# SilvioWeging/kASA

Measured on AMD Instinct MI355X. Metric: reads/s in identify (10M x 150bp vs k=12 index), higher is better.
Workload: dtype u64

## Files before the change

### kasa_amd/csrc/kasa_hip.hip

```cpp
#include <hip/hip_runtime.h>
#include <chrono>
#include <cstdlib>
#include <cstring>
#include <rocprim/device/device_radix_sort.hpp>
#include <rocprim/device/device_segmented_radix_sort.hpp>
#include <rocprim/iterator/transform_iterator.hpp>
#include <rocprim/device/device_scan.hpp>
#include <rocprim/functional.hpp>
#include <rocprim/iterator/counting_iterator.hpp>

#include <algorithm>
#include <cstdarg>
#include <cstdint>
#include <cstdio>
#include <cstring>
#include <map>
#include <mutex>
#include <new>
#include <string>
#include <thread>
#include <type_traits>
#include <vector>

#include <dlfcn.h>
// ... 1531 lines not shown
        if (p >= nQ) continue;
        const Key q = qv[it];
        uint32_t lo;
        Key eLo = 0, ePrev = 0;
        bool hasLo, hasPrev;
        if (staged) {
            const uint32_t a = pos[it];
            lo = ilo + a;
            hasLo = a < span; hasPrev = a > 0;
            if (hasLo) eLo = sIdx[a];
            if (hasPrev) ePrev = sIdx[a - 1];
            if (!hasPrev && lo > 0) { ePrev = idxKmer[lo - 1]; hasPrev = true; }
            if (!hasLo && lo < nIdx) { eLo = idxKmer[lo]; hasLo = true; }
        } else {
            lo = lower_bound_global<Key>(idxKmer, table, tb, q);
            hasLo = lo < nIdx; hasPrev = lo > 0;
            if (hasLo) eLo = idxKmer[lo];
            if (hasPrev) ePrev = idxKmer[lo - 1];
        }
        const Key xa = hasLo ? (q ^ eLo) : ~(Key)0;
        const Key xb = hasPrev ? (q ^ ePrev) : ~(Key)0;
        const int la = lcp_of_xor<Key>(xa);
        int L = lcp_of_xor<Key>(xa < xb ? xa : xb);
        const uint32_t r = (la == L) ? lo : lo - 1;
        int d = 0;
        if (L >= RANGE_LETTERS) {
            d = L > kHigh ? kHigh : L;
            const Key x = q ^ HAT_ALL;
            const Key z = ~(((x & LOW4_ALL) + LOW4_ALL) | x) & BIT4_ALL & hatLetters;
            if (z) {
                const int khat = KLETTERS - ((int)(8 * sizeof(Key)) - 5 - clz_key(z)) / 5;
                if (khat <= d) d = khat - 1;
            }
            if (d < kLow) d = 0;
        }
        outD[it] = (uint32_t)d;
        outRep[it] = r;
        const Key prevQ = it ? qv[it - 1] : qBefore;
        const int ql = (p == 0) ? 0 : lcp_letters<Key>(prevQ, q);
        uint32_t m = allLv;
        if (ql >= RANGE_LETTERS) m = (d > ql) ? ((((2u << (d - ql - 1)) - 1u) << (kHigh - d)) & allLv) : 0u;
        special[it] = m;
    }
    const uint32_t anySpecial = special[0] | special[1] | special[2] | special[3];
    for (int lv = 0; lv < nK; ++lv) {
        const bool has = (anySpecial >> lv) & 1u;
        const unsigned long long mk = __ballot(has);
        if (has && (mk & ((1ull << (tid & 63)) - 1ull)) == 0ull) {
            const uint32_t it = ((special[0] >> lv) & 1u) ? 0u : ((special[1] >> lv) & 1u) ? 1u : ((special[2] >> lv) & 1u) ? 2u : 3u;
            atomicMin(&sFirst[lv], p0 + it);
        }
    }
    if (fullTile) {
        *reinterpret_cast<uint4 *>(rep + p0) = make_uint4(outRep[0], outRep[1], outRep[2], outRep[3]);
        *reinterpret_cast<uchar4 *>(depth + p0) = make_uchar4((uint8_t)outD[0], (uint8_t)outD[1], (uint8_t)outD[2], (uint8_t)outD[3]);
    } else {
#pragma unroll
        for (int it = 0; it < ITEMS; ++it)
            if (p0 + it < nQ) { rep[p0 + it] = outRep[it]; depth[p0 + it] = (uint8_t)outD[it]; }
    }
    __syncthreads();
    if (tid < nK) tileFirst[(size_t)tid * nTiles + blockIdx.x] = sFirst[tid];
}

__device__ __forceinline__ void suffix_min_1024(uint32_t *sh, uint32_t v, uint32_t &excl, uint32_t &all)
{
    sh[threadIdx.x] = v;
    __syncthreads();
    for (int off = 1; off < 1024; off <<= 1) {
        const uint32_t o = (threadIdx.x >= (unsigned)off) ? sh[threadIdx.x - off] : NOPOS;
        __syncthreads();
        if (o < sh[threadIdx.x]) sh[threadIdx.x] = o;
        __syncthreads();
    }
    excl = (threadIdx.x == 0) ? NOPOS : sh[threadIdx.x - 1];
    all = sh[1023];
    __syncthreads();
}

__global__ __launch_bounds__(1024) void tile_suffix_local_kernel(const uint32_t *__restrict__ tileFirst, uint32_t *__restrict__ tileNext,
                                                                 uint32_t *__restrict__ chunkMin, uint32_t nTiles, uint32_t nChunks)
{
    __shared__ uint32_t sh[1024];
    const uint32_t lv = blockIdx.y, chunk = blockIdx.x;
    const uint64_t end = std::min<uint64_t>((uint64_t)(chunk + 1) * 1024u, nTiles);
    const int64_t t = (int64_t)end - 1 - threadIdx.x;
    const bool in = t >= (int64_t)chunk * 1024;
    uint32_t excl, all;
    suffix_min_1024(sh, in ? tileFirst[(size_t)lv * nTiles + t] : NOPOS, excl, all);
    if (in) tileNext[(size_t)lv * nTiles + t] = excl;
    if (threadIdx.x == 0) chunkMin[(size_t)lv * nChunks + chunk] = all;
}

__global__ __launch_bounds__(1024) void tile_suffix_kernel(const uint32_t *__restrict__ in0, uint32_t *__restrict__ out0,
                                                           uint32_t n, uint32_t last)
{
    __shared__ uint32_t sh[1024];
    const int lv = blockIdx.x;
    const uint32_t *in = in0 + (size_t)lv * n;
    uint32_t *out = out0 + (size_t)lv * n;
    uint32_t carry = last;
    for (int64_t hiT = (int64_t)n; hiT > 0; hiT -= 1024) {
        const int64_t t = hiT - 1 - threadIdx.x;
        uint32_t excl, all;
        suffix_min_1024(sh, (t >= 0) ? in[t] : NOPOS, excl, all);
        if (t >= 0) out[t] = excl < carry ? excl : carry;
        if (all < carry) carry = all;
    }
}

__global__ void tile_suffix_apply_kernel(uint32_t *__restrict__ tileNext, const uint32_t *__restrict__ chunkNext, uint32_t nTiles, uint32_t nChunks)
{
    const uint32_t t = blockIdx.x * blockDim.x + threadIdx.x, lv = blockIdx.y;
    if (t >= nTiles) return;
    const size_t at = (size_t)lv * nTiles + t;
    if (tileNext[at] == NOPOS) tileNext[at] = chunkNext[(size_t)lv * nChunks + (t >> 10)];
}

static int tile_suffix(kasa_ctx *c, uint32_t nTiles)
{
    if (nTiles == 0) return KASA_OK;
    const uint32_t nChunks = (nTiles + 1023u) / 1024u;
    int rc = c->tileChunks.reserve((size_t)2 * c->nK * nChunks * 4 + 64);
    if (rc) return rc;
    uint32_t *chunkMin = c->tileChunks.as<uint32_t>(), *chunkNext = chunkMin + (size_t)c->nK * nChunks;
    tile_suffix_local_kernel<<<dim3(nChunks, (unsigned)c->nK), 1024, 0, c->stream>>>(c->tileFirst.as<uint32_t>(), c->tileNext.as<uint32_t>(), chunkMin, nTiles, nChunks);
    tile_suffix_kernel<<<c->nK, 1024, 0, c->stream>>>(chunkMin, chunkNext, nChunks, (uint32_t)c->nQ);
    tile_suffix_apply_kernel<<<dim3(blocks_for(nTiles, 256), (unsigned)c->nK), 256, 0, c->stream>>>(c->tileNext.as<uint32_t>(), chunkNext, nTiles, nChunks);
    HIPCHK(hipGetLastError());
    return KASA_OK;
}

template <class Key>
__global__ void unique_flag_kernel(const Key *__restrict__ kmer, const uint32_t *__restrict__ read, uint32_t n, uint32_t *__restrict__ flag)
{
    const uint32_t i = blockIdx.x * blockDim.x + threadIdx.x;
    if (i < n) flag[i] = (i == 0 || kmer[i] != kmer[i - 1] || read[i] != read[i - 1]) ? 1u : 0u;
}

__global__ void read_count_kernel(const uint32_t *__restrict__ read, uint32_t n, uint64_t *__restrict__ cnt)
{
    const uint32_t i = blockIdx.x * blockDim.x + threadIdx.x;
    if (i < n) atomicAdd((unsigned long long *)&cnt[read[i]], 1ull);
}

template <class Key>
__global__ void unique_scatter_kernel(const Key *__restrict__ kmer, const uint32_t *__restrict__ read, uint32_t n,
                                      const uint32_t *__restrict__ slot, Key *__restrict__ outKmer, uint32_t *__restrict__ outRead)
{
    const uint32_t i = blockIdx.x * blockDim.x + threadIdx.x;
    if (i >= n) return;
    const uint32_t sl = slot[i];
    if (i == 0 || sl != slot[i - 1]) { outKmer[sl - 1] = kmer[i]; outRead[sl - 1] = read[i]; }
}

__global__ void slot_to_read_kernel(const uint32_t *__restrict__ slot, uint32_t n, const uint64_t *__restrict__ kmerOff, uint32_t nReads,
                                    uint32_t *__restrict__ read)
{
    const uint32_t i = blockIdx.x * blockDim.x + threadIdx.x;
    if (i >= n) return;
    const uint64_t s = slot[i];
    uint32_t lo = 0, hi = nReads;
    while (hi - lo > 1) { const uint32_t mid = lo + ((hi - lo) >> 1); if (kmerOff[mid] <= s) lo = mid; else hi = mid; }
    read[i] = lo;
}

template <class Key> static int lookup_part(kasa_ctx *c);

static constexpr unsigned SORT_TOP = 32, SORT_TOP_OLD = 40;
static constexpr uint32_t SORT_BUCKET_LIMIT = 1024;
static constexpr uint32_t SORT_BIG_CAP = 1u << 18;
static constexpr uint32_t SORT_BIG_LONGEST = 1u << 20;
static constexpr uint32_t RANK_TILE = 2048, RANK_HALO = 128;
template <class Key>
__global__ __launch_bounds__(256) void bucket_rank_kernel(const Key *__restrict__ kin, const uint32_t *__restrict__ vin, Key *__restrict__ kout,
                                                          uint32_t *__restrict__ vout, uint32_t n, int shift, uint32_t *__restrict__ big,
                                                          uint32_t *__restrict__ bigHead)
{
    constexpr uint32_t WIN = RANK_TILE + 2 * RANK_HALO;
    static_assert(WIN % 256 == 0, "whole wavefronts stage the window");
    __shared__ Key sK[WIN];
    __shared__ uint64_t sHead[WIN / 64];
    const uint32_t base = blockIdx.x * RANK_TILE;
    const uint32_t lo = base >= RANK_HALO ? base - RANK_HALO : 0u;
    const uint32_t hi = (uint64_t)base + RANK_TILE + RANK_HALO < (uint64_t)n ? base + RANK_TILE + RANK_HALO : n;
    const uint32_t win = hi - lo;
    for (uint32_t x = threadIdx.x; x < WIN; x += 256u) {
        bool head = false;
        if (x < win) {
            const uint32_t q = lo + x;
            const Key k = kin[q];
            head = q == 0u || (uint64_t)(kin[q - 1u] >> shift) != (uint64_t)(k >> shift);
            sK[x] = k;
        }
        const uint64_t m = __ballot(head);
        if ((threadIdx.x & 63u) == 0u) sHead[x >> 6] = m;
    }
    __syncthreads();
    const uint32_t lastWord = (win - 1u) >> 6;
    for (uint32_t e = threadIdx.x; e < RANK_TILE; e += 256u) {
        const uint32_t p = base + e;
        if (p >= n) break;
        const uint32_t i0 = p - lo, bit = i0 & 63u;
        const Key k = sK[i0];
        bool edge = false;
        uint32_t m = i0 >> 6;
        uint64_t w = sHead[m] & (~0ull >> (63u - bit));
        while (w == 0ull && m > 0u) w = sHead[--m];
        uint32_t hs = 0;
        if (w == 0ull) edge = true; else hs = m * 64u + 63u - (uint32_t)__clzll((long long)w);
        m = i0 >> 6;
        w = sHead[m] & ((~0ull << bit) << 1);
        while (w == 0ull && m < lastWord) w = sHead[++m];
        uint32_t he = win;
        if (w == 0ull) edge = edge || (hi < n); else he = m * 64u + (uint32_t)__ffsll((unsigned long long)w) - 1u;
        uint32_t L = i0 - hs, members = he - hs, rank = 0;
        if (!edge && members <= SORT_BUCKET_LIMIT) {
            for (uint32_t j = hs; j < i0; ++j) rank += (sK[j] <= k) ? 1u : 0u;
            for (uint32_t j = i0 + 1u; j < he; ++j) rank += (sK[j] < k) ? 1u : 0u;
        }
        if (edge) {
            const uint64_t top = (uint64_t)(k >> shift);
            uint32_t R = 0;
            rank = 0; L = 0;
            for (uint32_t q = p; q > 0 && L < SORT_BUCKET_LIMIT;) { --q; const Key o = kin[q]; if ((uint64_t)(o >> shift) != top) break; ++L; rank += (o <= k) ? 1u : 0u; }
            for (uint32_t q = p + 1; q < n && R < SORT_BUCKET_LIMIT; ++q) { const Key o = kin[q]; if ((uint64_t)(o >> shift) != top) break; ++R; rank += (o < k) ? 1u : 0u; }
            members = L + R + 1u;
        }
        if (members > SORT_BUCKET_LIMIT) {
            kout[p] = k; vout[p] = vin[p];
            if (L == 0u) { const uint32_t at = atomicAdd(big, 1u); if (at < SORT_BIG_CAP) bigHead[at] = p; }
        } else { const uint32_t at = p - L + rank; kout[at] = k; vout[at] = vin[p]; }
    }
}

__global__ __launch_bounds__(256) void bucket_rank32_kernel(const uint64_t *__restrict__ kin, const uint32_t *__restrict__ vin, uint64_t *__restrict__ kout,
                                                            uint32_t *__restrict__ vout, uint32_t n, int shift, uint32_t *__restrict__ big,
                                                            uint32_t *__restrict__ bigHead)
{
    constexpr uint32_t WIN = RANK_TILE + 2 * RANK_HALO, POS_BITS = 12;
    static_assert(WIN % 256 == 0 && WIN <= (1u << POS_BITS), "window positions fit the low bits of the LDS word; whole wavefronts stage it");
    __shared__ uint32_t sW[WIN + 1];
    __shared__ uint64_t sHead[WIN / 64];
    const uint32_t base = blockIdx.x * RANK_TILE;
    const uint32_t lo = base >= RANK_HALO ? base - RANK_HALO : 0u;
    const uint32_t hi = (uint64_t)base + RANK_TILE + RANK_HALO < (uint64_t)n ? base + RANK_TILE + RANK_HALO : n;
    const uint32_t win = hi - lo;
    const uint32_t lowMask = (1u << shift) - 1u;
    for (uint32_t x = threadIdx.x; x < WIN; x += 256u) {
        bool head = false;
        if (x < win) {
            const uint32_t q = lo + x;
            const uint64_t k = kin[q];
            head = q == 0u || (kin[q - 1u] >> shift) != (k >> shift);
            sW[x] = (((uint32_t)k & lowMask) << POS_BITS) | x;
        }
        const uint64_t m = __ballot(head);
        if ((threadIdx.x & 63u) == 0u) sHead[x >> 6] = m;
    }
    __syncthreads();
    const uint32_t lastWord = (win - 1u) >> 6;
    for (uint32_t e = threadIdx.x; e < RANK_TILE; e += 256u) {
        const uint32_t p = base + e;
        if (p >= n) break;
        const uint32_t i0 = p - lo, my = sW[i0], bit = i0 & 63u;
        bool edge = false;
        uint32_t m = i0 >> 6;
        uint64_t w = sHead[m] & (~0ull >> (63u - bit));
        while (w == 0ull && m > 0u) w = sHead[--m];
        uint32_t hs = 0;
        if (w == 0ull) edge = true; else hs = m * 64u + 63u - (uint32_t)__clzll((long long)w);
        m = i0 >> 6;
        w = sHead[m] & ((~0ull << bit) << 1);
        while (w == 0ull && m < lastWord) w = sHead[++m];
        uint32_t he = win;
        if (w == 0ull) edge = edge || (hi < n); else he = m * 64u + (uint32_t)__ffsll((unsigned long long)w) - 1u;
        uint32_t L = i0 - hs, members = he - hs, rank = 0;
        if (!edge && members <= SORT_BUCKET_LIMIT) {
            for (uint32_t j = hs; j < he; j += 2u) {
                const uint32_t a = sW[j], b = sW[j + 1u];
                rank += (a < my ? 1u : 0u) + ((j + 1u < he && b < my) ? 1u : 0u);
            }
        }
        const uint64_t k = kin[p];
        if (edge) {
            const uint64_t top = k >> shift;
            uint32_t R = 0;
            rank = 0; L = 0;
            for (uint32_t q = p; q > 0 && L < SORT_BUCKET_LIMIT;) { --q; const uint64_t o = kin[q]; if ((o >> shift) != top) break; ++L; rank += (o <= k) ? 1u : 0u; }
            for (uint32_t q = p + 1; q < n && R < SORT_BUCKET_LIMIT; ++q) { const uint64_t o = kin[q]; if ((o >> shift) != top) break; ++R; rank += (o < k) ? 1u : 0u; }
            members = L + R + 1u;
        }
        if (members > SORT_BUCKET_LIMIT) {
            kout[p] = k; vout[p] = vin[p];
            if (L == 0u) { const uint32_t at = atomicAdd(big, 1u); if (at < SORT_BIG_CAP) bigHead[at] = p; }
        } else { const uint32_t at = p - L + rank; kout[at] = k; vout[at] = vin[p]; }
    }
}

__global__ __launch_bounds__(256) void bucket_rank64_kernel(const uint64_t *__restrict__ kin, const uint32_t *__restrict__ vin, uint64_t *__restrict__ kout,
                                                            uint32_t *__restrict__ vout, uint32_t n, int shift, uint32_t *__restrict__ big,
                                                            uint32_t *__restrict__ bigHead)
{
    constexpr uint32_t WIN = RANK_TILE + 2 * RANK_HALO, POS_BITS = 12;
    static_assert(WIN % 256 == 0 && WIN <= (1u << POS_BITS), "window positions fit the low bits of the LDS word; whole wavefronts stage it");
    __shared__ __attribute__((aligned(16))) uint64_t sW[WIN + 2];
    __shared__ uint64_t sHead[WIN / 64];
    const uint32_t base = blockIdx.x * RANK_TILE;
    const uint32_t lo = base >= RANK_HALO ? base - RANK_HALO : 0u;
    const uint32_t hi = (uint64_t)base + RANK_TILE + RANK_HALO < (uint64_t)n ? base + RANK_TILE + RANK_HALO : n;
    const uint32_t win = hi - lo;
    const uint64_t lowMask = (1ull << shift) - 1ull;
    for (uint32_t x = threadIdx.x; x < WIN; x += 256u) {
        bool head = false;
        if (x < win) {
            const uint32_t q = lo + x;
            const uint64_t k = kin[q];
            head = q == 0u || (kin[q - 1u] >> shift) != (k >> shift);
            sW[x] = ((k & lowMask) << POS_BITS) | x;
        }
        const uint64_t m = __ballot(head);
        if ((threadIdx.x & 63u) == 0u) sHead[x >> 6] = m;
    }
    __syncthreads();
    const uint32_t lastWord = (win - 1u) >> 6;
    for (uint32_t e = threadIdx.x; e < RANK_TILE; e += 256u) {
        const uint32_t p = base + e;
        if (p >= n) break;
        const uint32_t i0 = p - lo, bit = i0 & 63u;
        const uint64_t my = sW[i0];
        bool edge = false;
        uint32_t m = i0 >> 6;
        uint64_t w = sHead[m] & (~0ull >> (63u - bit));
        while (w == 0ull && m > 0u) w = sHead[--m];
        uint32_t hs = 0;
        if (w == 0ull) edge = true; else hs = m * 64u + 63u - (uint32_t)__clzll((long long)w);
        m = i0 >> 6;
        w = sHead[m] & ((~0ull << bit) << 1);
        while (w == 0ull && m < lastWord) w = sHead[++m];
        uint32_t he = win;
        if (w == 0ull) edge = edge || (hi < n); else he = m * 64u + (uint32_t)__ffsll((unsigned long long)w) - 1u;
        uint32_t L = i0 - hs, members = he - hs, rank = 0;
        if (!edge && members <= SORT_BUCKET_LIMIT) {
            uint32_t j = hs;
            if (j & 1u) { rank += sW[j] < my ? 1u : 0u; ++j; }
            for (; j + 1u < he; j += 2u) {
                const ulonglong2 ab = *reinterpret_cast<const ulonglong2 *>(&sW[j]);
                rank += (ab.x < my ? 1u : 0u) + (ab.y < my ? 1u : 0u);
            }
            if (j < he) rank += sW[j] < my ? 1u : 0u;
        }
        const uint64_t k = kin[p];
        if (edge) {
            const uint64_t top = k >> shift;
            uint32_t R = 0;
            rank = 0; L = 0;
            for (uint32_t q = p; q > 0 && L < SORT_BUCKET_LIMIT;) { --q; const uint64_t o = kin[q]; if ((o >> shift) != top) break; ++L; rank += (o <= k) ? 1u : 0u; }
            for (uint32_t q = p + 1; q < n && R < SORT_BUCKET_LIMIT; ++q) { const uint64_t o = kin[q]; if ((o >> shift) != top) break; ++R; rank += (o < k) ? 1u : 0u; }
            members = L + R + 1u;
        }
        if (members > SORT_BUCKET_LIMIT) {
            kout[p] = k; vout[p] = vin[p];
            if (L == 0u) { const uint32_t at = atomicAdd(big, 1u); if (at < SORT_BIG_CAP) bigHead[at] = p; }
        } else { const uint32_t at = p - L + rank; kout[at] = k; vout[at] = vin[p]; }
    }
}

template <class Key>
__global__ void bucket_bounds_kernel(const Key *__restrict__ kin, uint32_t n, int shift, const uint32_t *__restrict__ head, uint32_t nHead,
                                     uint32_t *__restrict__ begin, uint32_t *__restrict__ end, uint32_t *__restrict__ longest)
{
    const uint32_t x = blockIdx.x * blockDim.x + threadIdx.x;
    if (x >= nHead) return;
    const uint32_t p = head[x];
    const uint64_t top = (uint64_t)(kin[p] >> shift);
    uint32_t lo = p, hi = n;
    while (lo < hi) { const uint32_t mid = lo + ((hi - lo) >> 1); if ((uint64_t)(kin[mid] >> shift) <= top) lo = mid + 1; else hi = mid; }
    begin[x] = p; end[x] = lo;
    atomicMax(longest, lo - p);
}

template <class Key>
static int sort_and_range_impl(kasa_ctx *c, int unique)
{
    c->grouped = false; c->slotOf = nullptr;
    HIPCHK(hipSetDevice(c->ix->device));
    uint64_t nQ = c->nQ;
    int rc;
    if ((rc = c->qKmerB.reserve(nQ * sizeof(Key) + 64)) || (rc = c->qReadB.reserve(nQ * 4 + 64))) return rc;
    Span stage(c, c->timers[KASA_STAGE_SORT]); if ((rc = stage.begin())) return rc;
    if (nQ > 0) {
        const unsigned BITS = (unsigned)KeyTraits<Key>::BITS;
        auto radix = [&](DevBuf &kIn, DevBuf &vIn, DevBuf &kOut, DevBuf &vOut, unsigned lo, unsigned hi) -> int {
            return dev_sort_pairs(c->sortTmp, c->stream, kIn.as<Key>(), kOut.as<Key>(), vIn.as<uint32_t>(), vOut.as<uint32_t>(), (size_t)nQ, lo, hi);
        };
        if (c->debugFlags & 64) {
            if ((rc = radix(c->qKmerA, c->qReadA, c->qKmerB, c->qReadB, 0u, BITS))) return rc;
        } else {
            const unsigned top = ((sizeof(Key) == 8) != ((c->debugFlags & 2097152) != 0)) ? SORT_TOP : SORT_TOP_OLD;
            uint32_t *big = &c->ctr()->sortBig.count, *longest = &c->ctr()->sortBig.longest;
            if ((rc = c->sortBig.reserve((size_t)SORT_BIG_CAP * 12 + 64))) return rc;
            uint32_t *bigHead = c->sortBig.as<uint32_t>(), *segBegin = bigHead + SORT_BIG_CAP, *segEnd = segBegin + SORT_BIG_CAP;
            if (c->debugFlags & 512) {
                if ((rc = radix(c->qKmerA, c->qReadA, c->qKmerB, c->qReadB, BITS - top, BITS))) return rc;
            } else {
                if ((rc = c->sortTmp.reserve(kasa_radix::scratch_bytes<Key>(nQ)))) return rc;
                Key *kRes; uint32_t *vRes;
                Span passes(c, c->kernels[KASA_KERNEL_SORT_PASSES]); if ((rc = passes.begin())) return rc;
                HIPCHK(kasa_radix::sort_pairs<Key>(c->qKmerA.as<Key>(), c->qReadA.as<uint32_t>(), c->qKmerB.as<Key>(), c->qReadB.as<uint32_t>(), (uint32_t)nQ,
                                                   (int)(BITS - top), (int)top, c->sortTmp.p, c->stream, &kRes, &vRes, (c->debugFlags & 524288) ? kasa_radix::MODE_FIRST : 0));
                if ((rc = passes.end())) return rc;
                if (kRes == c->qKmerA.as<Key>() && (top / 8) % 2 == 0) { std::swap(c->qKmerA, c->qKmerB); std::swap(c->qReadA, c->qReadB); }
                if (kRes != c->qKmerB.as<Key>()) return fail(KASA_E_HIP, "query sort: unexpected result buffer");
            }
            HIPCHK(hipMemsetAsync(&c->ctr()->sortBig, 0, sizeof(LongBuckets), c->stream));
            Span rank(c, c->kernels[KASA_KERNEL_BUCKET_RANK]); if ((rc = rank.begin())) return rc;
            static_assert(KeyTraits<uint64_t>::BITS - SORT_TOP_OLD + 12 <= 32, "bucket_rank32_kernel: low key bits and window position share a word");
            static_assert(KeyTraits<uint64_t>::BITS - SORT_TOP + 12 <= 52, "bucket_rank64_kernel: low key bits and window position share a word");
            if (sizeof(Key) == 8 && top != SORT_TOP_OLD && !(c->debugFlags & 4194304))
                bucket_rank64_kernel<<<blocks_for(nQ, RANK_TILE), 256, 0, c->stream>>>(c->qKmerB.as<uint64_t>(), c->qReadB.as<uint32_t>(), c->qKmerA.as<uint64_t>(),
                                                                                      c->qReadA.as<uint32_t>(), (uint32_t)nQ, (int)(BITS - top), big, bigHead);
            else if (sizeof(Key) == 8 && top != SORT_TOP_OLD)
                bucket_rank_kernel<Key><<<blocks_for(nQ, RANK_TILE), 256, 0, c->stream>>>(c->qKmerB.as<Key>(), c->qReadB.as<uint32_t>(), c->qKmerA.as<Key>(),
                                                                                          c->qReadA.as<uint32_t>(), (uint32_t)nQ, (int)(BITS - top), big, bigHead);
            else if constexpr (sizeof(Key) == 8)
                bucket_rank32_kernel<<<blocks_for(nQ, RANK_TILE), 256, 0, c->stream>>>(c->qKmerB.as<uint64_t>(), c->qReadB.as<uint32_t>(), c->qKmerA.as<uint64_t>(),
                                                                                      c->qReadA.as<uint32_t>(), (uint32_t)nQ, (int)(BITS - top), big, bigHead);
            else
                bucket_rank_kernel<Key><<<blocks_for(nQ, RANK_TILE), 256, 0, c->stream>>>(c->qKmerB.as<Key>(), c->qReadB.as<uint32_t>(), c->qKmerA.as<Key>(),
                                                                                          c->qReadA.as<uint32_t>(), (uint32_t)nQ, (int)(BITS - top), big, bigHead);
            HIPCHK(hipGetLastError());
            if ((rc = rank.end())) return rc;
            uint32_t hBig = 0;
            if ((rc = fetch(c->stream, hBig, big))) return rc;
            if (hBig) {
                uint32_t hLongest = 0;
                if (hBig <= SORT_BIG_CAP) {
                    bucket_bounds_kernel<Key><<<blocks_for(hBig, 256), 256, 0, c->stream>>>(c->qKmerB.as<Key>(), (uint32_t)nQ, (int)(BITS - top), bigHead, hBig,
                                                                                         segBegin, segEnd, longest);
                    HIPCHK(hipGetLastError());
                    if ((rc = fetch(c->stream, hLongest, longest))) return rc;
                }
                if (hBig <= SORT_BIG_CAP && hLongest <= SORT_BIG_LONGEST && !(c->debugFlags & 128)) {
                    if ((rc = dev_segmented_sort_pairs(c->sortTmp, c->stream, c->qKmerB.as<Key>(), c->qKmerA.as<Key>(), c->qReadB.as<uint32_t>(), c->qReadA.as<uint32_t>(),
                                                       (unsigned)nQ, hBig, segBegin, segEnd, 0u, BITS - top))) return rc;
                } else if ((rc = radix(c->qKmerB, c->qReadB, c->qKmerA, c->qReadA, 0u, BITS))) return rc;
            }
            std::swap(c->qKmerA, c->qKmerB);
            std::swap(c->qReadA, c->qReadB);
        }
    }
    c->qKmer = c->qKmerB.p;
    c->qRead = c->qReadB.as<uint32_t>();
    if (c->payloadIsSlot && nQ > 0) {
        if (unique) {
            slot_to_read_kernel<<<blocks_for(nQ, 256), 256, 0, c->stream>>>(c->qReadB.as<uint32_t>(), (uint32_t)nQ, c->kmerOff.as<uint64_t>(), (uint32_t)c->nReads, c->qReadA.as<uint32_t>());
            HIPCHK(hipMemcpyAsync(c->qReadB.p, c->qReadA.p, nQ * 4, hipMemcpyDeviceToDevice, c->stream));
            c->payloadIsSlot = false;
        } else c->slotOf = c->qReadB.as<uint32_t>();
    }
    if (unique && nQ > 1) {
        if ((rc = c->rep.reserve(nQ * 4 + 64))) return rc;
        uint32_t *slot = c->rep.as<uint32_t>();
        unique_flag_kernel<Key><<<blocks_for(nQ, 256), 256, 0, c->stream>>>(c->keys<Key>(), c->qRead, (uint32_t)nQ, slot);
        if ((rc = dev_inclusive_scan(c->sortTmp, c->stream, slot, slot, (size_t)nQ, rocprim::plus<uint32_t>()))) return rc;
        unique_scatter_kernel<Key><<<blocks_for(nQ, 256), 256, 0, c->stream>>>(c->keys<Key>(), c->qRead, (uint32_t)nQ, slot,
            c->qKmerA.as<Key>(), c->qReadA.as<uint32_t>());
        HIPCHK(hipGetLastError());
        uint32_t kept = 0;
        if ((rc = fetch(c->stream, kept, slot + (nQ - 1)))) return rc;
        nQ = c->nQ = kept; c->uniqueDone = true;
        HIPCHK(hipMemcpyAsync(c->qKmerB.p, c->qKmerA.p, nQ * sizeof(Key), hipMemcpyDeviceToDevice, c->stream));
        HIPCHK(hipMemcpyAsync(c->qReadB.p, c->qReadA.p, nQ * 4, hipMemcpyDeviceToDevice, c->stream));
        uint64_t *ko = c->kmerOff.as<uint64_t>();
        HIPCHK(hipMemsetAsync(ko, 0, ((size_t)c->nReads + 1) * 8, c->stream));
        read_count_kernel<<<blocks_for(nQ, 256), 256, 0, c->stream>>>(c->qReadB.as<uint32_t>(), (uint32_t)nQ, ko);
        if ((rc = dev_exclusive_scan(c->sortTmp, c->stream, ko, ko, (uint64_t)0, (size_t)c->nReads + 1, rocprim::plus<uint64_t>()))) return rc;
    }
    if ((rc = stage.end())) return rc;
    return lookup_part<Key>(c);
}

template <class Key>
static int lookup_part(kasa_ctx *c)
{
    const uint64_t nQ = c->nQ;
    int rc;
    if ((rc = c->depth.reserve(nQ + 64)) || (rc = c->rep.reserve(nQ * 4 + 64))) return rc;
    const uint32_t nTiles = (uint32_t)((nQ + TILE - 1) / TILE);
    if ((rc = c->tileFirst.reserve((size_t)c->nK * (nTiles + 1) * 4)) || (rc = c->tileNext.reserve((size_t)c->nK * (nTiles + 1) * 4)) ||
        (rc = c->tileBounds.reserve(((size_t)nTiles + 1) * 8)))
        return rc;

    Span stage(c, c->timers[KASA_STAGE_LOOKUP]); if ((rc = stage.begin())) return rc;
    if (nQ > 0) {
        Span kernel(c, c->kernels[KASA_KERNEL_LOOKUP]);
        if (c->lookupMode == 1) {
            if ((rc = kernel.begin())) return rc;
            lookup_kernel<Key><<<nTiles, TILE_THREADS, 0, c->stream>>>(c->keys<Key>(), (uint32_t)nQ, c->ix->kmer.as<Key>(), (uint32_t)c->ix->n,
                c->ix->table.as<uint32_t>(), c->ix->tb, c->kHigh, c->kLow, c->depth.as<uint8_t>(), c->rep.as<uint32_t>(),
                c->tileFirst.as<uint32_t>(), nTiles);
        } else {
            tile_bounds_kernel<Key><<<blocks_for(2ull * nTiles, 256), 256, 0, c->stream>>>(c->keys<Key>(), (uint32_t)nQ, c->ix->kmer.as<Key>(),
                c->ix->table.as<uint32_t>(), c->ix->tb, nTiles, c->tileBounds.as<uint32_t>());
            if ((rc = kernel.begin())) return rc;
            lookup_tile_kernel<Key><<<nTiles, TILE_THREADS, 0, c->stream>>>(c->keys<Key>(), (uint32_t)nQ, c->ix->kmer.as<Key>(), (uint32_t)c->ix->n,
                c->ix->table.as<uint32_t>(), c->ix->tb, c->tileBounds.as<uint32_t>(), c->kHigh, c->kLow, c->depth.as<uint8_t>(),
                c->rep.as<uint32_t>(), c->tileFirst.as<uint32_t>(), nTiles);
        }
        HIPCHK(hipGetLastError());
        if ((rc = kernel.end())) return rc;
        if ((rc = tile_suffix(c, nTiles))) return rc;
    }
    if ((rc = stage.end())) return rc;
    c->state = 3;
    return KASA_OK;
}

extern "C" int kasa_batch_sort_and_range(kasa_ctx *c, int unique)
{
    if (!c) return fail(KASA_E_ARG, "ctx is NULL");
    if (c->state < 2) return fail(KASA_E_STATE, "kasa_batch_sort_and_range: batch not encoded");
    return c->ix->wide ? sort_and_range_impl<key128>(c, unique) : sort_and_range_impl<uint64_t>(c, unique);
}

static constexpr int GITEMS = 2;
static constexpr int GTHREADS = TILE / GITEMS;
static constexpr int GOVF = 1024;
static constexpr int GSPAN = 3072;
static constexpr uint32_t GMARGIN = 96;

static constexpr uint32_t SEG_TAX_MASK = (1u << 22) - 1u;
static constexpr uint32_t REC_SPLIT = 1u << 29;
static constexpr uint32_t REC_SAT = 1u << 30;
template <int RW> struct RecTraits;
template <> struct RecTraits<8> { static constexpr int LEVELS = 8, INL = 4, SEG0 = 4, OBITS = 3; };
template <> struct RecTraits<16> { static constexpr int LEVELS = 25, INL = 8, SEG0 = 8, OBITS = 5; };
__device__ __forceinline__ bool seg_covers(uint32_t s, uint32_t k) { return ((s >> 22) & 31u) <= k && k <= (s >> 27); }
__device__ __forceinline__ uint32_t seg_level_mask(uint32_t s, int kHigh)
{
    const int lvLo = kHigh - (int)(s >> 27), lvHi = kHigh - (int)((s >> 22) & 31u);
    return ((2u << lvHi) - 1u) & ~((1u << lvLo) - 1u);
}
template <int RW> __device__ __forceinline__ uint32_t rec_nseg(const uint32_t *w, const uint32_t *__restrict__ pool)
{
    if constexpr (RW == 8) { const uint32_t n = w[3] & 255u; return n == 255u ? pool[w[7]] : n; }
    else return w[3];
}
static constexpr uint32_t POOL_SIZES = 4;
template <int RW> __device__ __forceinline__ uint32_t rec_seg(const uint32_t *w, const uint32_t *__restrict__ pool, uint32_t nseg, uint32_t i)
{
    typedef RecTraits<RW> RT;
    if (nseg <= (uint32_t)RT::INL || i < (uint32_t)RT::INL - 1u) return w[RT::SEG0 + i];
    const uint32_t skip = (RW == 8 && (w[2] & REC_SAT)) ? POOL_SIZES : 0u;
    return pool[w[RT::SEG0 + RT::INL - 1] + 1u + skip + i - ((uint32_t)RT::INL - 1u)];
}

__device__ __forceinline__ uint32_t special_mask(int ql, int d, int kHigh, uint32_t allLv)
{
    if (ql < RANGE_LETTERS) return allLv;
    return (d > ql) ? ((((2u << (d - ql - 1)) - 1u) << (kHigh - d)) & allLv) : 0u;
}

__device__ __forceinline__ uint32_t block_excl_prefix_sum(uint32_t v, uint32_t *sh, uint32_t &total)
{
    const int t = threadIdx.x, lane = t & 63, wv = t >> 6;
    uint32_t incl = v;
    incl = wave_incl_sum(incl);
    if (lane == 63) sh[wv] = incl;
    __syncthreads();
    uint32_t before = 0, all = 0;
    for (int w = 0; w < GTHREADS / 64; ++w) { const uint32_t o = sh[w]; if (w < wv) before += o; all += o; }
    total = all;
    __syncthreads();
    return before + incl - v;
}

template <class Meta, class GetMeta, class GetTax, class Emit>
__device__ __forceinline__ bool walk_segments(uint32_t j, int d, int kLow, GetMeta meta, GetTax tax, uint32_t nIdx, Emit emit, uint32_t maxSteps = 0xFFFFFFFFu)
{
    constexpr int LM = sizeof(Meta) == 1 ? 15 : 255, DS = sizeof(Meta) == 1 ? 4 : 8;
    const int gLow = group_letters(kLow);
    auto one = [&](uint32_t i, int kLast, uint32_t m) {
        const int dup = (int)(m >> DS);
        const int kFirst = dup < RANGE_LETTERS ? kLow : (dup + 1 > kLow ? dup + 1 : kLow);
        if (kFirst <= kLast) emit(tax(i) | ((uint32_t)kFirst << 22) | ((uint32_t)kLast << 27));
    };
    const uint32_t mj = meta(j);
    one(j, d, mj);
    const int chain0 = d > RANGE_LETTERS ? d : RANGE_LETTERS;
    uint32_t li = j, ri = j + 1;
    uint32_t mli = mj;
    uint32_t mri = ri < nIdx ? (uint32_t)meta(ri) : 0u;
    int lc = li > 0 ? ((int)(mli & LM) < chain0 ? (int)(mli & LM) : chain0) : -1;
    int rc = ri < nIdx ? ((int)(mri & LM) < chain0 ? (int)(mri & LM) : chain0) : -1;
    uint32_t steps = 0;
    while (lc >= gLow || rc >= gLow) {
        if (++steps > maxSteps) return false;
        if (lc >= rc) {
            --li;
            mli = meta(li);
            one(li, lc < d ? lc : d, mli);
            const int l = (int)(mli & LM);
            lc = li > 0 ? (l < lc ? l : lc) : -1;
        } else {
            one(ri, rc < d ? rc : d, mri);
            ++ri;
            if (ri < nIdx) { mri = meta(ri); const int l = (int)(mri & LM); rc = l < rc ? l : rc; } else rc = -1;
        }
    }
    return true;
}

#define KASA_DPP_ID(v, ctrl, rows, id) __builtin_amdgcn_update_dpp((int)(id), (int)(v), (ctrl), (rows), 0xf, false)
__device__ __forceinline__ int wave_incl_min(int v)
{
    constexpr int TOP = 0x7fffffff;
    { const int o = KASA_DPP_ID(v, 0x111, 0xf, TOP); v = o < v ? o : v; }
    { const int o = KASA_DPP_ID(v, 0x112, 0xf, TOP); v = o < v ? o : v; }
    { const int o = KASA_DPP_ID(v, 0x114, 0xf, TOP); v = o < v ? o : v; }
    { const int o = KASA_DPP_ID(v, 0x118, 0xf, TOP); v = o < v ? o : v; }
    { const int o = KASA_DPP_ID(v, 0x142, 0xa, TOP); v = o < v ? o : v; }
    { const int o = KASA_DPP_ID(v, 0x143, 0xc, TOP); v = o < v ? o : v; }
    return v;
}
__device__ __forceinline__ int wave_max_int(int v) { return ~__builtin_amdgcn_readlane(wave_incl_min(~v), 63); }
template <class Meta, class F>
__device__ __forceinline__ void coop_walk(const Meta *__restrict__ meta, const uint32_t *__restrict__ tax, uint32_t nIdx, uint32_t j, int d, int kLow, int lane, F f)
{
    constexpr int LM = sizeof(Meta) == 1 ? 15 : 255;
    const int gLow = group_letters(kLow);
    const int chain0 = d > RANGE_LETTERS ? d : RANGE_LETTERS;
    const uint32_t lastIdx = nIdx - 1u;
    int run = chain0;
    {
        auto load = [&](uint32_t a0, uint32_t &mc, uint32_t &mo, uint32_t &tx) {
            const uint32_t a = a0 + (uint32_t)lane;
            const uint32_t idx = a <= j ? j - a : 0u;
            mc = (uint32_t)meta[idx < lastIdx ? idx + 1u : lastIdx]; mo = (uint32_t)meta[idx]; tx = tax[idx];
        };
        uint32_t mc, mo, tx, mcN = 0, moN = 0, txN = 0;
        load(1u, mc, mo, tx);
        for (uint32_t a0 = 1;; a0 += 64) {
            load(a0 + 64u, mcN, moN, txN);
            const uint32_t a = a0 + (uint32_t)lane;
            const bool valid = a <= j;
            const uint32_t idx = valid ? j - a : 0u;
            int v = wave_incl_min(valid ? (int)(mc & (uint32_t)LM) : -1);
            v = v < run ? v : run;
            const bool ok = valid && v >= gLow;
            f(ok, idx, v, 0, mo, tx);
            if (__ballot(ok) != ~0ull) break;
            run = __builtin_amdgcn_readlane(v, 63);
            mc = mcN; mo = moN; tx = txN;
        }
    }
    run = chain0;
    {
        auto load = [&](uint32_t b0, uint32_t &mo, uint32_t &tx) {
            const uint32_t idx0 = j + b0 + (uint32_t)lane;
            const uint32_t idx = (idx0 < nIdx && idx0 > j) ? idx0 : 0u;
            mo = (uint32_t)meta[idx]; tx = tax[idx];
        };
        uint32_t mo, tx, moN = 0, txN = 0;
        load(1u, mo, tx);
        for (uint32_t b0 = 1;; b0 += 64) {
            load(b0 + 64u, moN, txN);
            const uint32_t idx = j + b0 + (uint32_t)lane;
            const bool valid = idx < nIdx && idx > j;
            int v = wave_incl_min(valid ? (int)(mo & (uint32_t)LM) : -1);
            v = v < run ? v : run;
            const bool ok = valid && v >= gLow;
            f(ok, idx, v, 1, mo, tx);
            if (__ballot(ok) != ~0ull) break;
            run = __builtin_amdgcn_readlane(v, 63);
            mo = moN; tx = txN;
        }
    }
}
static constexpr uint32_t LONG_STEPS = 48, LONG_STEPS_CROWDED = 8;

struct ProfLayout {
    uint32_t tb, nb, lb;
    __host__ __device__ uint32_t bits() const { return tb + nb + lb; }
};
static inline ProfLayout prof_layout(uint32_t nTaxa, int nK)
{
    ProfLayout L;
    L.tb = 1; while ((1u << L.tb) <= nTaxa) ++L.tb;
    L.nb = L.tb < 13 ? L.tb : 13;
    L.lb = 1; while ((1u << L.lb) < (uint32_t)nK) ++L.lb;
    return L;
}
__device__ __forceinline__ uint64_t profile_key_of(uint32_t lv, uint32_t n, uint32_t tax, uint32_t hits, ProfLayout L)
{
    const uint64_t f = ((uint64_t)lv << (L.tb + L.nb)) | ((uint64_t)n << L.tb) | tax;
    return (f << 16) | hits;
}
__device__ __forceinline__ void fixed_add(uint64_t *hiTab, uint64_t *midTab, uint64_t *loTab, size_t cell, uint64_t c, uint32_t n)
{
    if (n == 1) { atomicAdd((unsigned long long *)&hiTab[cell], (unsigned long long)c); return; }
    uint64_t R = 0xFFFFFFFFFFFFFFFFull / n;
    if ((n & (n - 1)) == 0) R += 1;
    const uint64_t lo64 = c * R;
    const uint64_t hi = __umul64hi(c, R);
    const uint64_t lo = lo64 & 0xFFFFFFFFull, mid = lo64 >> 32;
    if (lo) atomicAdd((unsigned long long *)&loTab[cell], (unsigned long long)lo);
    if (mid) atomicAdd((unsigned long long *)&midTab[cell], (unsigned long long)mid);
    if (hi) atomicAdd((unsigned long long *)&hiTab[cell], (unsigned long long)hi);
}

__device__ __forceinline__ uint32_t lvp_rows(int levels) { return (uint32_t)(levels + 3) / 2u; }
__device__ __forceinline__ uint32_t lvp_unit(int lv) { return (lv & 1) ? 0x10000u : 1u; }
__device__ __forceinline__ uint32_t lvp_get(const uint32_t *col, int stride, int lv) { return (col[(lv >> 1) * stride] >> (16 * (lv & 1))) & 0xFFFFu; }
template <class F> __device__ __forceinline__ void lvp_running(uint32_t *col, int stride, int nK, F f)
{
    uint32_t running = 0;
    for (int w = 0; 2 * w < nK; ++w) {
        const uint32_t x = col[w * stride];
        const int lo = (int)(int16_t)(x & 0xFFFFu);
        const int hi = (int)(int16_t)((x - (uint32_t)lo) >> 16);
// ... 5911 lines not shown
```

Baseline: 59.92 million.

## Restructure bucket rank kernel around wavefront rows with 32-bit LDS keys

The bucket_rank64 kernel now stages each 64-key row per wavefront, keeping keys and values in registers, finding head flags with shuffles rather than a second global load, and storing only 32-bit low key bits in LDS. Nearest bucket heads outside a row are precomputed per row, which replaces the per-thread while-loop scans, and the rank count reads four keys per LDS load with a position-aware tie-break instead of packing positions into 64-bit words. The goal is less global and LDS traffic and fewer divergent loops in the post-sort ranking step. The cost is tighter assumptions (halo of exactly 128, low bits under 32) and more complex boundary logic.

After: 60.66 million, median of 6. 1.01x the previous value.

```diff
diff --git a/kasa_amd/csrc/kasa_hip.hip b/kasa_amd/csrc/kasa_hip.hip
--- a/kasa_amd/csrc/kasa_hip.hip
+++ b/kasa_amd/csrc/kasa_hip.hip
@@ -1857,67 +1857,113 @@
                                                             uint32_t *__restrict__ vout, uint32_t n, int shift, uint32_t *__restrict__ big,
                                                             uint32_t *__restrict__ bigHead)
 {
-    constexpr uint32_t WIN = RANK_TILE + 2 * RANK_HALO, POS_BITS = 12;
-    static_assert(WIN % 256 == 0 && WIN <= (1u << POS_BITS), "window positions fit the low bits of the LDS word; whole wavefronts stage it");
-    __shared__ __attribute__((aligned(16))) uint64_t sW[WIN + 2];
-    __shared__ uint64_t sHead[WIN / 64];
+    constexpr uint32_t WIN = RANK_TILE + 2 * RANK_HALO, ROWS = WIN / 64, PER = RANK_TILE / 256, NONE = ~0u;
+    static_assert(RANK_TILE % 256 == 0 && RANK_HALO == 128, "four wavefronts share the tile's rows and take one of the four halo rows each");
+    __shared__ __attribute__((aligned(16))) uint32_t sLow[WIN];
+    __shared__ uint64_t sHead[ROWS];
+    __shared__ uint32_t sBefore[ROWS], sAfter[ROWS];
     const uint32_t base = blockIdx.x * RANK_TILE;
-    const uint32_t lo = base >= RANK_HALO ? base - RANK_HALO : 0u;
-    const uint32_t hi = (uint64_t)base + RANK_TILE + RANK_HALO < (uint64_t)n ? base + RANK_TILE + RANK_HALO : n;
-    const uint32_t win = hi - lo;
-    const uint64_t lowMask = (1ull << shift) - 1ull;
-    for (uint32_t x = threadIdx.x; x < WIN; x += 256u) {
-        bool head = false;
-        if (x < win) {
-            const uint32_t q = lo + x;
-            const uint64_t k = kin[q];
-            head = q == 0u || (kin[q - 1u] >> shift) != (k >> shift);
-            sW[x] = ((k & lowMask) << POS_BITS) | x;
-        }
+    const uint32_t lane = threadIdx.x & 63u, wave = (uint32_t)__builtin_amdgcn_readfirstlane((int)(threadIdx.x >> 6));
+    const int64_t origin = (int64_t)base - RANK_HALO, end = (int64_t)n;
+    const uint32_t lowMask = (uint32_t)((1ull << shift) - 1ull);
+    const uint32_t row0 = RANK_HALO / 64u + wave * PER;
+    const uint32_t rowH = wave < 2u ? wave : RANK_TILE / 64u + wave;
+
+    uint64_t k[PER], kH = 0ull, before0 = 0ull, beforeH = 0ull;
+    uint32_t v[PER];
+#pragma unroll
+    for (uint32_t j = 0; j < PER; ++j) {
+        const int64_t q = origin + (row0 + j) * 64u + lane;
+        const bool in = q < end;
+        k[j] = in ? kin[q] : 0ull;
+        v[j] = in ? vin[q] : 0u;
+    }
+    {
+        const int64_t q = origin + rowH * 64u + lane, b0 = origin + row0 * 64u - 1, bH = origin + rowH * 64u - 1;
+        if (q >= 0 && q < end) kH = kin[q];
+        if (b0 >= 0 && b0 < end) before0 = kin[b0];
+        if (bH >= 0 && bH < end) beforeH = kin[bH];
+    }
+    auto stage = [&](uint32_t row, uint64_t key, uint64_t before) -> uint64_t {
+        const int64_t q = origin + row * 64u + lane;
+        const bool in = q >= 0 && q < end;
+        const uint32_t pl = (uint32_t)__shfl_up((int)(uint32_t)key, 1), ph = (uint32_t)__shfl_up((int)(uint32_t)(key >> 32), 1);
+        const uint64_t prev = lane == 0u ? before : ((uint64_t)ph << 32) | pl;
+        const bool head = in ? (q == 0 || ((prev ^ key) >> shift) != 0ull) : q == end;
+        if (in) sLow[row * 64u + lane] = (uint32_t)key & lowMask;
         const uint64_t m = __ballot(head);
-        if ((threadIdx.x & 63u) == 0u) sHead[x >> 6] = m;
-    }
+        if (lane == 0u) sHead[row] = m;
+        return ((uint64_t)(uint32_t)__builtin_amdgcn_readlane((int)(uint32_t)(key >> 32), 63) << 32) | (uint32_t)__builtin_amdgcn_readlane((int)(uint32_t)key, 63);
+    };
+    stage(rowH, kH, beforeH);
+#pragma unroll
+    for (uint32_t j = 0; j < PER; ++j) before0 = stage(row0 + j, k[j], before0);
     __syncthreads();
-    const uint32_t lastWord = (win - 1u) >> 6;
-    for (uint32_t e = threadIdx.x; e < RANK_TILE; e += 256u) {
-        const uint32_t p = base + e;
-        if (p >= n) break;
-        const uint32_t i0 = p - lo, bit = i0 & 63u;
-        const uint64_t my = sW[i0];
-        bool edge = false;
-        uint32_t m = i0 >> 6;
-        uint64_t w = sHead[m] & (~0ull >> (63u - bit));
-        while (w == 0ull && m > 0u) w = sHead[--m];
-        uint32_t hs = 0;
-        if (w == 0ull) edge = true; else hs = m * 64u + 63u - (uint32_t)__clzll((long long)w);
-        m = i0 >> 6;
-        w = sHead[m] & ((~0ull << bit) << 1);
-        while (w == 0ull && m < lastWord) w = sHead[++m];
-        uint32_t he = win;
-        if (w == 0ull) edge = edge || (hi < n); else he = m * 64u + (uint32_t)__ffsll((unsigned long long)w) - 1u;
+    if (wave == 0u) {
+        for (uint32_t row = lane; row < ROWS; row += 64u) {
+            uint32_t at = NONE;
+            for (uint32_t m = row; m > 0u && at == NONE;) { const uint64_t w = sHead[--m]; if (w != 0ull) at = m * 64u + 63u - (uint32_t)__clzll((long long)w); }
+            sBefore[row] = at;
+        }
+    } else if (wave == 1u) {
+        for (uint32_t row = lane; row < ROWS; row += 64u) {
+            uint32_t at = NONE;
+            for (uint32_t m = row + 1u; m < ROWS && at == NONE; ++m) { const uint64_t w = sHead[m]; if (w != 0ull) at = m * 64u + (uint32_t)__ffsll((unsigned long long)w) - 1u; }
+            sAfter[row] = at;
+        }
+    }
+    __syncthreads();
+
+    const bool cut = origin + (int64_t)WIN < end;
+    const uint32_t winEnd = cut ? WIN : (uint32_t)(end - origin);
+    const uint64_t upToMe = ~0ull >> (63u - lane), aboveMe = (~0ull << lane) << 1;
+    const uint4 *sLow4 = reinterpret_cast<const uint4 *>(sLow);
+#pragma unroll
+    for (uint32_t j = 0; j < PER; ++j) {
+        const uint32_t row = row0 + j, i0 = row * 64u + lane;
+        const int64_t q = origin + i0;
+        if (q >= end) break;
+        const uint32_t p = (uint32_t)q;
+        const uint64_t key = k[j], hw = sHead[row];
+        const uint64_t heads = ((uint64_t)(uint32_t)__builtin_amdgcn_readfirstlane((int)(uint32_t)(hw >> 32)) << 32) | (uint32_t)__builtin_amdgcn_readfirstlane((int)(uint32_t)hw);
+        const uint32_t farBefore = (uint32_t)__builtin_amdgcn_readfirstlane((int)sBefore[row]), farAfter = (uint32_t)__builtin_amdgcn_readfirstlane((int)sAfter[row]);
+        const uint64_t below = heads & upToMe, above = heads & aboveMe;
+        const uint32_t hs = below != 0ull ? row * 64u + 63u - (uint32_t)__clzll((long long)below) : farBefore;
+        const uint32_t he = above != 0ull ? row * 64u + (uint32_t)__ffsll((unsigned long long)above) - 1u : farAfter != NONE ? farAfter : winEnd;
+        const bool edge = hs == NONE || (above == 0ull && farAfter == NONE && cut);
         uint32_t L = i0 - hs, members = he - hs, rank = 0;
         if (!edge && members <= SORT_BUCKET_LIMIT) {
-            uint32_t j = hs;
-            if (j & 1u) { rank += sW[j] < my ? 1u : 0u; ++j; }
-            for (; j + 1u < he; j += 2u) {
-                const ulonglong2 ab = *reinterpret_cast<const ulonglong2 *>(&sW[j]);
-                rank += (ab.x < my ? 1u : 0u) + (ab.y < my ? 1u : 0u);
-            }
-            if (j < he) rank += sW[j] < my ? 1u : 0u;
-        }
-        const uint64_t k = kin[p];
+            const uint32_t my = (uint32_t)key & lowMask, up = my + 1u;
+            const uint32_t qa = hs >> 2, qm = i0 >> 2, qb = (he - 1u) >> 2;
+            auto ragged = [&](uint32_t g, uint32_t limit) -> uint32_t {
+                const uint4 t = sLow4[g];
+                const uint32_t d = g * 4u - hs;
+                return ((d < members && t.x < limit) ? 1u : 0u) + ((d + 1u < members && t.y < limit) ? 1u : 0u) +
+                       ((d + 2u < members && t.z < limit) ? 1u : 0u) + ((d + 3u < members && t.w < limit) ? 1u : 0u);
+            };
+            rank = ragged(qa, qa < qm ? up : my) + ragged(qb, qb != qa ? my : 0u);
+#pragma unroll 1
+            for (uint32_t g = qa + 1u; g < qb; ++g) {
+                const uint4 t = sLow4[g];
+                const uint32_t limit = g < qm ? up : my;
+                rank += (t.x < limit ? 1u : 0u) + (t.y < limit ? 1u : 0u) + (t.z < limit ? 1u : 0u) + (t.w < limit ? 1u : 0u);
+            }
+            const uint4 t = sLow4[qm];
+            const uint32_t c = i0 & 3u, f = qm * 4u;
+            rank += ((c > 0u && f >= hs && t.x == my) ? 1u : 0u) + ((c > 1u && f + 1u >= hs && t.y == my) ? 1u : 0u) + ((c > 2u && f + 2u >= hs && t.z == my) ? 1u : 0u);
+        }
         if (edge) {
-            const uint64_t top = k >> shift;
+            const uint64_t top = key >> shift;
             uint32_t R = 0;
             rank = 0; L = 0;
-            for (uint32_t q = p; q > 0 && L < SORT_BUCKET_LIMIT;) { --q; const uint64_t o = kin[q]; if ((o >> shift) != top) break; ++L; rank += (o <= k) ? 1u : 0u; }
-            for (uint32_t q = p + 1; q < n && R < SORT_BUCKET_LIMIT; ++q) { const uint64_t o = kin[q]; if ((o >> shift) != top) break; ++R; rank += (o < k) ? 1u : 0u; }
+            for (uint32_t o = p; o > 0 && L < SORT_BUCKET_LIMIT;) { --o; const uint64_t other = kin[o]; if ((other >> shift) != top) break; ++L; rank += (other <= key) ? 1u : 0u; }
+            for (uint32_t o = p + 1; o < n && R < SORT_BUCKET_LIMIT; ++o) { const uint64_t other = kin[o]; if ((other >> shift) != top) break; ++R; rank += (other < key) ? 1u : 0u; }
             members = L + R + 1u;
         }
         if (members > SORT_BUCKET_LIMIT) {
-            kout[p] = k; vout[p] = vin[p];
+            kout[p] = key; vout[p] = v[j];
             if (L == 0u) { const uint32_t at = atomicAdd(big, 1u); if (at < SORT_BIG_CAP) bigHead[at] = p; }
-        } else { const uint32_t at = p - L + rank; kout[at] = k; vout[at] = vin[p]; }
+        } else { const uint32_t at = p - L + rank; kout[at] = key; vout[at] = v[j]; }
     }
 }
 
@@ -1971,7 +2017,7 @@
             HIPCHK(hipMemsetAsync(&c->ctr()->sortBig, 0, sizeof(LongBuckets), c->stream));
             Span rank(c, c->kernels[KASA_KERNEL_BUCKET_RANK]); if ((rc = rank.begin())) return rc;
             static_assert(KeyTraits<uint64_t>::BITS - SORT_TOP_OLD + 12 <= 32, "bucket_rank32_kernel: low key bits and window position share a word");
-            static_assert(KeyTraits<uint64_t>::BITS - SORT_TOP + 12 <= 52, "bucket_rank64_kernel: low key bits and window position share a word");
+            static_assert(KeyTraits<uint64_t>::BITS - SORT_TOP < 32, "bucket_rank64_kernel: the low key bits are a 32-bit word, and that word + 1 does not wrap");
             if (sizeof(Key) == 8 && top != SORT_TOP_OLD && !(c->debugFlags & 4194304))
                 bucket_rank64_kernel<<<blocks_for(nQ, RANK_TILE), 256, 0, c->stream>>>(c->qKmerB.as<uint64_t>(), c->qReadB.as<uint32_t>(), c->qKmerA.as<uint64_t>(),
                                                                                       c->qReadA.as<uint32_t>(), (uint32_t)nQ, (int)(BITS - top), big, bigHead);
```
